# Ipsedo/MARLClassification

Hardware: NVIDIA B200
Metric: image_episodes_per_sec (higher is better)
Workload: dtype tf32x3

## Files before the change

include/marlc.h:

```cpp
#ifndef MARLC_H
#define MARLC_H
#include <stddef.h>
#include <stdint.h>
#ifdef __cplusplus
extern "C" {
#endif

#define MARLC_MAX_ACTIONS 16
#define MARLC_MAX_CNN_LAYERS 6

int marlc_version(void);
const char* marlc_last_error(void);
long marlc_selftest_fastdiv(int d_max, int stride);


int marlc_patch_gather(const float* img, const int64_t* pos, float* obs, int Na, int B, int C, int H, int W, int f,
                       void* stream);
int marlc_patch_gather_backward(const float* d_obs, const int64_t* pos, float* d_img, int Na, int B, int C, int H,
                                int W, int f, void* stream);

int marlc_transition(int64_t* pos, const int64_t* act, const int64_t* table, int nA, int M, int f, int H, int W,
                     float* norm_pos, int* err_flag, void* stream);

int marlc_normalized_positions(const int64_t* pos, float* out, int M, int H, int W, void* stream);
// ... 39 lines not shown
} marlc_config;

typedef struct marlc_engine marlc_engine;

int marlc_engine_create(const marlc_config* cfg, marlc_engine** out);
void marlc_engine_destroy(marlc_engine* e);

typedef struct marlc_plan {
    int cnn_wide;
    int cnn_nw;
    int cnn_batches;
    int cnn_ctas;
    int cnn_passes;
    int cnn_tail;
    int lstm_tc;
    int lstm_hu;
    int lstm_bn;
    int lstm_fat;
    int lstm_ks;
    int lstm_ksplit;
    int lstm_tail_rows;
    int sweep_chained;
    int staged_step_pre, staged_step_post, staged_bwd_pre, staged_bwd_post;
} marlc_plan;
int marlc_engine_plan(const marlc_engine* e, marlc_plan* out);

int marlc_engine_param_count(const marlc_engine* e);
int marlc_engine_param_info(const marlc_engine* e, int idx, char* name, int64_t* offset, int* ndim, int64_t* shape);
int64_t marlc_engine_param_floats(const marlc_engine* e);

size_t marlc_engine_workspace_bytes(const marlc_engine* e);
int marlc_engine_bind(marlc_engine* e, void* workspace, float* params, float* grads);
int marlc_engine_buffer(const marlc_engine* e, const char* name, size_t* offset, size_t* nbytes);

int marlc_episode_forward(marlc_engine* e, const float* img, const int64_t* pos0, const float* const* hidden0,
                          const int64_t* actions, void* stream);
int marlc_model_step(marlc_engine* e, const float* patch, const float* msg, const float* npos,
                     const float* const* hidden, void* stream);
int marlc_engine_seed(marlc_engine* e, uint64_t seed, void* stream);

int marlc_loss_phase_a(marlc_engine* e, const int64_t* targets, void* stream);
int marlc_loss_phase_b(marlc_engine* e, void* stream);

int marlc_episode_backward(marlc_engine* e, const float* img, int accumulate, void* stream);

int marlc_episode_image_grad(marlc_engine* e, float* d_img, void* stream);
// ... 20 lines not shown
```

marlclassification_b200/_lib.py:

```python
from __future__ import annotations

import ctypes as C
import os

import torch

from . import _build

MAX_ACTIONS = 16
MAX_CNN_LAYERS = 6


class MarlcConfig(C.Structure):

    _fields_ = [
        ("na", C.c_int), ("nb", C.c_int), ("T", C.c_int), ("C", C.c_int), ("H", C.c_int), ("W", C.c_int),
        ("f", C.c_int), ("n_actions", C.c_int), ("actions", (C.c_int * 2) * MAX_ACTIONS),
        ("cnn_layers", C.c_int), ("cnn_cin", C.c_int * MAX_CNN_LAYERS), ("cnn_cout", C.c_int * MAX_CNN_LAYERS),
        ("cnn_groups", C.c_int * MAX_CNN_LAYERS),
        ("n_b", C.c_int), ("n_a", C.c_int), ("n_m", C.c_int), ("n_m_o", C.c_int), ("n_d", C.c_int),
        ("nl_b", C.c_int), ("nl_a", C.c_int), ("nb_class", C.c_int),
        ("gamma", C.c_float), ("use_tc", C.c_int), ("use_chains", C.c_int),
    ]


class MarlcPlan(C.Structure):

    _fields_ = [(name, C.c_int) for name in (
        "cnn_wide", "cnn_nw", "cnn_batches", "cnn_ctas", "cnn_passes", "cnn_tail",
        "lstm_tc", "lstm_hu", "lstm_bn", "lstm_fat", "lstm_ks", "lstm_ksplit", "lstm_tail_rows",
        "sweep_chained", "staged_step_pre", "staged_step_post", "staged_bwd_pre", "staged_bwd_post")]

    def as_dict(self) -> dict:
        return {name: getattr(self, name) for name, _ in self._fields_}


_P = C.c_void_p
_SIGS = {
    "marlc_version": (C.c_int, []),
    "marlc_selftest_fastdiv": (C.c_long, [C.c_int, C.c_int]),
    "marlc_last_error": (C.c_char_p, []),
    "marlc_patch_gather": (C.c_int, [_P, _P, _P] + [C.c_int] * 6 + [_P]),
    "marlc_patch_gather_backward": (C.c_int, [_P, _P, _P] + [C.c_int] * 6 + [_P]),
    "marlc_transition": (C.c_int, [_P, _P, _P] + [C.c_int] * 5 + [_P, _P, _P]),
    "marlc_normalized_positions": (C.c_int, [_P, _P, C.c_int, C.c_int, C.c_int, _P]),
    "marlc_images_u8_to_f32": (C.c_int, [_P, _P] + [C.c_int] * 5 + [_P]),
    "marlc_linear": (C.c_int, [_P, _P, _P, _P, C.c_int, C.c_int, C.c_int, _P]),
    "marlc_ln_silu": (C.c_int, [_P, _P, _P, _P, C.c_int, C.c_int, _P]),
    "marlc_msg_mean": (C.c_int, [_P, _P, C.c_int, C.c_int, C.c_int, _P]),
    "marlc_tc_gemm": (C.c_int, [_P, C.c_int64, C.c_int, _P, C.c_int64, C.c_int, _P, C.c_int64, _P, C.c_int64, C.c_int, _P,
                                _P, C.c_int64, C.c_int, C.c_int, C.c_int, C.c_int, C.c_int, C.c_int, _P]),
    "marlc_tc_lstm_pair": (C.c_int, [_P, C.c_int, C.c_int, C.c_int] + [C.POINTER(_P)] * 9 + [C.c_int, _P]),
    "marlc_split_lo": (C.c_int, [_P, _P, C.c_int64, _P]),
    "marlc_tc_lstm_pair_presplit": (C.c_int, [_P, _P, C.c_int, C.c_int, C.c_int] + [C.POINTER(_P)] * 13 + [_P]),
# ... 81 lines not shown
```

marlclassification_b200/csrc/chain.cu:

```cuda
#include <initializer_list>

#include <stdlib.h>

#include "chain.cuh"
#include "cnn_wide.cuh"

namespace marlc {

constexpr int RB = 4;
constexpr int CT = 256;
constexpr int WT_K = 16;
constexpr int WT_P = WT_K + 1;
constexpr float LN_EPS_C = 1e-5f;


__device__ void rb_linear(const float* xT, const float* __restrict__ W, const float* __restrict__ bias, float* ys,
                          int ldy, int N, int K, float* wt) {
    const int tid = threadIdx.x;
    const bool vec = ((K & 3) == 0) && (((uintptr_t)W & 15) == 0);
    for (int n0 = 0; n0 < N; n0 += CT) {
        float acc[RB];
#pragma unroll
        for (int r = 0; r < RB; ++r) acc[r] = 0.f;
        const int n = n0 + tid;
// ... 49 lines not shown
#pragma unroll
        for (int r = 0; r < RB; ++r) out[r * ldo + k] = acc[r];
    }
    __syncthreads();
}


__device__ __forceinline__ void stage_w(float* dst, const float* __restrict__ W, int N, int K, int P) {
    stage_rows(dst, W, N, K, P);
}
__host__ __device__ inline int odd_pitch(int K) { return K | 1; }

__device__ __forceinline__ bool stage_w_async(float* dst, const float* __restrict__ W, int N, int K) {
    if (((K & 3) != 0) || ((reinterpret_cast<uintptr_t>(W) & 15) != 0)) { stage_rows(dst, W, N, K, K); return false; }
    const int tot4 = (N * K) >> 2;
    const uint32_t d0 = (uint32_t)__cvta_generic_to_shared(dst);
    for (int i = threadIdx.x; i < tot4; i += CT)
        asm volatile("cp.async.cg.shared.global [%0], [%1], 16;" ::"r"(d0 + 16u * i), "l"(W + 4 * (long)i) : "memory");
    asm volatile("cp.async.commit_group;" ::: "memory");
    return true;
}
__device__ __forceinline__ void stage_wait_all() { asm volatile("cp.async.wait_group 0;" ::: "memory"); }

__device__ void rb_linear_s(const float* xT, const float* Ws, int P, const float* __restrict__ bias, float* ys, int ldy,
                            int N, int K) {
    for (int n = threadIdx.x; n < N; n += CT) {
        const float* w = Ws + n * P;
        float a0 = 0.f, a1 = 0.f, a2 = 0.f, a3 = 0.f;
#pragma unroll 4
        for (int k = 0; k < K; ++k) {
            const float wv = w[k];
            const float4 x = *reinterpret_cast<const float4*>(xT + k * RB);
            a0 = fmaf(wv, x.x, a0); a1 = fmaf(wv, x.y, a1); a2 = fmaf(wv, x.z, a2); a3 = fmaf(wv, x.w, a3);
        }
        const float b = bias ? bias[n] : 0.f;
        ys[n] = a0 + b; ys[ldy + n] = a1 + b; ys[2 * ldy + n] = a2 + b; ys[3 * ldy + n] = a3 + b;
    }
    __syncthreads();
}

__device__ void rb_dx_s(const float* dyT, const float* Ws, int P, float* out, int ldo, int N, int K) {
    for (int k = threadIdx.x; k < K; k += CT) {
        float a0 = 0.f, a1 = 0.f, a2 = 0.f, a3 = 0.f;
#pragma unroll 4
        for (int n = 0; n < N; ++n) {
            const float wv = Ws[n * P + k];
            const float4 d = *reinterpret_cast<const float4*>(dyT + n * RB);
            a0 = fmaf(wv, d.x, a0); a1 = fmaf(wv, d.y, a1); a2 = fmaf(wv, d.z, a2); a3 = fmaf(wv, d.w, a3);
        }
        out[k] = a0; out[ldo + k] = a1; out[2 * ldo + k] = a2; out[3 * ldo + k] = a3;
    }
    __syncthreads();
}

__device__ void rb_ln_silu(const float* ys, int ldy, int N, const float* __restrict__ gamma,
                           const float* __restrict__ beta, int rows_valid, long row0, float* pre_g, long ld_pre,
                           float* s_g, long ld_s, float* sT, float* s_lo = nullptr) {
    const int warp = threadIdx.x >> 5, lane = threadIdx.x & 31;
    if (warp < RB) {
        const int r = warp;
        if (r < rows_valid) {
            const float* y = ys + r * ldy;
            const float inv = 1.0f / (float)N;
            float s = 0.f;
            for (int n = lane; n < N; n += 32) s += y[n];
            const float mean = warp_sum(s) * inv;
            float v = 0.f;
            for (int n = lane; n < N; n += 32) { const float d = y[n] - mean; v += d * d; }
            const float rstd = 1.0f / sqrtf(warp_sum(v) * inv + LN_EPS_C);
            for (int n = lane; n < N; n += 32) {
                const float yv = y[n];
                if (pre_g) pre_g[(row0 + r) * ld_pre + n] = yv;
                const float o = siluf_((yv - mean) * rstd * gamma[n] + beta[n]);
                if (s_g) s_g[(row0 + r) * ld_s + n] = o;
                if (s_lo) s_lo[(row0 + r) * ld_s + n] = tf32_lo(o);
                if (sT) sT[n * RB + r] = o;
            }
        } else if (sT) {
            for (int n = lane; n < N; n += 32) sT[n * RB + r] = 0.f;
        }
    }
    __syncthreads();
}

__device__ void rb_ln_silu_bwd(float* ds, float* ypre, int ld, int N, const float* __restrict__ gamma,
                               const float* __restrict__ beta, int rows_valid, long row0, float* dy, float* dyT,
                               float* dy_g, long ld_dyg, float* dgamma, float* dbeta, float* dbias) {
    const int warp = threadIdx.x >> 5, lane = threadIdx.x & 31;
    if (warp < RB) {
        const int r = warp;
        float* y = ypre + r * ld;
        float* g = ds + r * ld;
        if (r < rows_valid) {
            const float inv = 1.0f / (float)N;
            float s = 0.f;
            for (int n = lane; n < N; n += 32) s += y[n];
            const float mean = warp_sum(s) * inv;
            float v = 0.f;
            for (int n = lane; n < N; n += 32) { const float d = y[n] - mean; v += d * d; }
            const float rstd = 1.0f / sqrtf(warp_sum(v) * inv + LN_EPS_C);
            float c1 = 0.f, c2 = 0.f;
            for (int n = lane; n < N; n += 32) {
// ... 68 lines not shown
}
static int maxw_of(std::initializer_list<int> v) {
    int m = 4;
    for (int x : v) m = max(m, x);
    return (m + 3) & ~3;
}
ChainStage step_pre_stage(int n_m, int n1, int n2, int nd) {
    const int maxw = maxw_of({n_m, n1, n2, nd});
    return {maxw, staged_floats(maxw, n1, odd_pitch(n_m), n2, odd_pitch(n1))};
}
ChainStage step_post_stage(int n1, int n2) {
    const int maxw = maxw_of({n1, n2});
    return {maxw, staged_floats(maxw, n2, odd_pitch(n1), 0, 0)};
}
ChainStage bwd_pre_stage(int n_m, int n1, int nb) {
    const int maxw = maxw_of({n_m, n1, nb});
    return {maxw, staged_floats(maxw, n_m, n1, n1, nb)};
}
ChainStage bwd_post_stage(int n_m, int n1, int n2) {
    const int maxw = maxw_of({n_m, n1, n2});
    return {maxw, staged_floats(maxw, n2, n1, n1, n_m)};
}

struct StepPreWideArgs { StepPreArgs a; int maxw; int staged; int cnn_blocks; int dec_blocks; int trig; CnnWidePlan wide; };

__global__ void __launch_bounds__(CT, 1) step_pre_wide_kernel(const StepPreWideArgs ka) {
    extern __shared__ __align__(16) float sm[];
    const StepPreArgs& a = ka.a;
    if (ka.trig) pdl_trigger();
    if ((int)blockIdx.x < ka.cnn_blocks) {
        cnn_fwd_wide(a.cnn, ka.wide, blockIdx.x, ka.cnn_blocks, sm);
        return;
    }
    const int db = (int)blockIdx.x - ka.cnn_blocks;
    const int nrb = (a.M + RB - 1) / RB;
    const int n_m = a.d0.n_in, n1 = a.d0.n_out, n2 = a.d3.n_out;
    ChainSmem S(sm, ka.maxw);
    const int P0 = odd_pitch(n_m), P3 = odd_pitch(n1);
    float* W0s = S.wres;
    float* W3s = W0s + n1 * P0;
    const int tid = threadIdx.x;
    const bool fast = ka.staged && RB * n_m <= CT && n1 <= CT && n2 <= CT && 2 * (n1 + n2) <= CT * WT_P;
    float* sG0 = S.wt;
    float* sB0 = sG0 + n1;
    float* sG3 = sB0 + n1;
    float* sB3 = sG3 + n2;
    const int mr = tid / n_m, mj = tid - mr * n_m;
    auto load_mean = [&](int rb) -> float {
        const int row0 = rb * RB;
        return (tid < RB * n_m && rb < nrb && row0 + mr < a.M) ? other_agents_mean(a.msg_in, row0 + mr, mj, a.Na, a.Nb, n_m) : 0.f;
    };
    if (fast) {
        float g0 = 0.f, b0 = 0.f, g3 = 0.f, b3 = 0.f;
        if (tid < n1) { g0 = a.d0.g[tid]; b0 = a.d0.be[tid]; }
        if (tid < n2) { g3 = a.d3.g[tid]; b3 = a.d3.be[tid]; }
        stage_w(W0s, a.d0.W, n1, n_m, P0);
        stage_w(W3s, a.d3.W, n2, n1, P3);
        if (tid < n1) { sG0[tid] = g0; sB0[tid] = b0; }
        if (tid < n2) { sG3[tid] = g3; sB3[tid] = b3; }
    } else if (ka.staged) {
        stage_w(W0s, a.d0.W, n1, n_m, P0);
        stage_w(W3s, a.d3.W, n2, n1, P3);
    }
    pdl_wait();
    float mv = fast ? load_mean(db) : 0.f;
    for (int rb = db; rb < nrb; rb += ka.dec_blocks) {
        const int row0 = rb * RB;
        const int rows_valid = min(RB, a.M - row0);
        if (fast) {
            if (tid < RB * n_m) {
                if (mr < rows_valid) a.coll[(long)(row0 + mr) * n_m + mj] = mv;
                S.bufT[mj * RB + mr] = mv;
            }
            __syncthreads();
            mv = load_mean(rb + ka.dec_blocks);
            rb_linear_s(S.bufT, W0s, P0, a.d0.b, S.bufA, ka.maxw, n1, n_m);
            rb_ln_silu(S.bufA, ka.maxw, n1, sG0, sB0, rows_valid, row0, a.dec_y1, n1, a.dec_s1, n1, S.bufT);
            rb_linear_s(S.bufT, W3s, P3, a.d3.b, S.bufA, ka.maxw, n2, n1);
            rb_ln_silu(S.bufA, ka.maxw, n2, sG3, sB3, rows_valid, row0, a.dec_y2, n2, a.U + a.F, a.ldu, nullptr,
                       a.U_lo ? a.U_lo + a.F : nullptr);
        } else {
            for (int e = tid; e < RB * n_m; e += CT) {
                const int r = e / n_m, j = e % n_m;
                float v = 0.f;
                if (r < rows_valid) {
                    v = other_agents_mean(a.msg_in, row0 + r, j, a.Na, a.Nb, n_m);
                    a.coll[(long)(row0 + r) * n_m + j] = v;
                }
                S.bufT[j * RB + r] = v;
            }
            __syncthreads();
            if (ka.staged) rb_linear_s(S.bufT, W0s, P0, a.d0.b, S.bufA, ka.maxw, n1, n_m);
            else rb_linear(S.bufT, a.d0.W, a.d0.b, S.bufA, ka.maxw, n1, n_m, S.wt);
            rb_ln_silu(S.bufA, ka.maxw, n1, a.d0.g, a.d0.be, rows_valid, row0, a.dec_y1, n1, a.dec_s1, n1, S.bufT);
            if (ka.staged) rb_linear_s(S.bufT, W3s, P3, a.d3.b, S.bufA, ka.maxw, n2, n1);
            else rb_linear(S.bufT, a.d3.W, a.d3.b, S.bufA, ka.maxw, n2, n1, S.wt);
            rb_ln_silu(S.bufA, ka.maxw, n2, a.d3.g, a.d3.be, rows_valid, row0, a.dec_y2, n2, a.U + a.F, a.ldu, nullptr,
                       a.U_lo ? a.U_lo + a.F : nullptr);
        }
        {
            const int warp = tid >> 5, lane = tid & 31, nd = a.pos.n_out;
            if (warp < rows_valid) {
                const long m = row0 + warp;
                const float p0 = a.npos[2 * m], p1 = a.npos[2 * m + 1];
                const float inv = 1.0f / (float)nd;
                float sum = 0.f;
                for (int j = lane; j < nd; j += 32) {
                    const float y = fmaf(p1, a.pos.W[2 * j + 1], p0 * a.pos.W[2 * j]) + a.pos.b[j];
                    a.pos_y[m * nd + j] = y;
                    S.bufB[warp * ka.maxw + j] = y;
                    sum += y;
                }
                const float mean = warp_sum(sum) * inv;
                float v = 0.f;
                for (int j = lane; j < nd; j += 32) { const float d = S.bufB[warp * ka.maxw + j] - mean; v += d * d; }
                const float rstd = 1.0f / sqrtf(warp_sum(v) * inv + LN_EPS_C);
                float* o = a.U + m * a.ldu + a.F + n2;
                float* ol = a.U_lo ? a.U_lo + m * a.ldu + a.F + n2 : nullptr;
                for (int j = lane; j < nd; j += 32) {
                    const float v2 = siluf_((S.bufB[warp * ka.maxw + j] - mean) * rstd * a.pos.g[j] + a.pos.be[j]);
                    o[j] = v2;
                    if (ol) ol[j] = tf32_lo(v2);
                }
            }
        }
        __syncthreads();
    }
}

static int persistent_blocks(int nrb, size_t smem_bytes, int waves = 1) {
    const int per_sm = (int)max((size_t)1, min((size_t)8, (size_t)(220 * 1024) / max(smem_bytes, (size_t)1)));
    return max(1, min(nrb, MARLC_SMS * per_sm * waves));
}

static int step_pre_small(const StepPreArgs& a, cudaStream_t s);

constexpr int CNN_WIDE_MIN = 256;
StepPrePlan step_pre_plan(const CnnDesc& d, bool have_img, bool have_wT, int M, CnnWidePlan* wide) {
    CnnWidePlan w;
    memset(&w, 0, sizeof(w));
    if (M >= CNN_WIDE_MIN) w = cnn_wide_plan(d, have_img, have_wT);
    if (wide) *wide = w;
    StepPrePlan p;
    p.nw = w.ok ? CW_NW : 1;
    p.cnn_blocks = w.ok ? min((M + CW_NW - 1) / CW_NW, MARLC_SMS) : 0;
    return p;
}

int step_pre(const StepPreArgs& a, cudaStream_t s) {
    if (a.M <= 0) return 0;
    static_assert(CW_THREADS == CT, "the wide feature extractor runs inside the chain kernel's CTA shape");
    StepPreWideArgs ka;
    const StepPrePlan pl = step_pre_plan(a.cnn.d, a.cnn.img != nullptr && a.cnn.patch == nullptr, true, a.M, &ka.wide);
    if (!ka.wide.ok) return step_pre_small(a, s);
    ka.a = a;
    const ChainStage st = step_pre_stage(a.d0.n_in, a.d0.n_out, a.d3.n_out, a.pos.n_out);
    ka.maxw = st.maxw;
    const int wfl = st.wfl;
    ka.staged = wfl > 0;
    ka.cnn_blocks = pl.cnn_blocks;
    const size_t smem = max(chain_smem_bytes(ka.maxw) + sizeof(float) * (size_t)wfl, sizeof(float) * (size_t)ka.wide.smem_floats);
    MARLC_CHECK(smem <= 226 * 1024, "step_pre: shared memory %zu B too large", smem);
    static size_t attr = 0;
    if (smem > 48 * 1024 && smem > attr) {
        MARLC_CUDA(cudaFuncSetAttribute(step_pre_wide_kernel, cudaFuncAttributeMaxDynamicSharedMemorySize, (int)smem));
        attr = smem;
    }
    ka.dec_blocks = persistent_blocks((a.M + RB - 1) / RB, smem);
    const int grid = ka.cnn_blocks + ka.dec_blocks;
    ka.trig = pdl_trigger_early();
    MARLC_CUDA(launch_pdl(step_pre_wide_kernel, dim3(grid), dim3(CT), smem, s, ka));
    MARLC_LAUNCH_CHECK();
    return 0;
}

struct StepPreKernelArgs { StepPreArgs a; int maxw; int staged; int trig; };

__global__ void __launch_bounds__(CT) step_pre_kernel(const StepPreKernelArgs ka) {
    extern __shared__ __align__(16) float sm[];
    const StepPreArgs& a = ka.a;
    if (ka.trig) pdl_trigger();
    if ((int)blockIdx.x < a.M) {
        cnn_fwd_block(a.cnn, blockIdx.x, sm);
        return;
    }
    const int row0 = ((int)blockIdx.x - a.M) * RB;
    const int rows_valid = min(RB, a.M - row0);
    const int n_m = a.d0.n_in, n1 = a.d0.n_out, n2 = a.d3.n_out;
    ChainSmem S(sm, ka.maxw);
    const int P0 = odd_pitch(n_m), P3 = odd_pitch(n1);
    float* W0s = S.wres;
    float* W3s = W0s + n1 * P0;
    if (ka.staged && RB * n_m <= CT && n1 <= CT && n2 <= CT && 2 * (n1 + n2) <= CT * WT_P) {
        float* sG0 = S.wt;
// ... 197 lines not shown
    if (lane == 0) {
        float pa = 0.f;
        for (int j = 0; j < p.nA; ++j) {
            const float pr = logit[j] * invd;
            p.probs[(long)m * p.nA + j] = pr;
            if (j == act) pa = pr;
        }
        p.logp[m] = logf(pa);
        p.act_out[m] = act;
        int py = p.pos_in[2 * m], px = p.pos_in[2 * m + 1];
        if (act >= 0 && act < p.nA) {
            const int ny = py + p.moves[2 * act], nx = px + p.moves[2 * act + 1];
            if ((ny >= 0) & (ny + p.f < p.H) & (nx >= 0) & (nx + p.f < p.W)) { py = ny; px = nx; }
        }
        p.pos_out[2 * m] = py; p.pos_out[2 * m + 1] = px;
        p.step_pos[2 * (long)m] = py; p.step_pos[2 * (long)m + 1] = px;
        p.npos_out[2 * m] = (float)py / (float)p.H;
        p.npos_out[2 * m + 1] = (float)px / (float)p.W;
    }
}

struct StepPostKernelArgs { StepPostArgs a; int maxw; int pol_blocks; int staged; int trig; };

__global__ void __launch_bounds__(CT) step_post_kernel(const StepPostKernelArgs ka) {
    extern __shared__ __align__(16) float sm[];
    const StepPostArgs& a = ka.a;
    if (ka.trig) pdl_trigger();
    if ((int)blockIdx.x < ka.pol_blocks) {
        const int warp = threadIdx.x >> 5;
        const int m = blockIdx.x * (CT / 32) + warp;
        pdl_wait();
        if (m < a.M) policy_tail_row(a, m, sm + warp * a.act.nl);
        return;
    }
    const int row0 = ((int)blockIdx.x - ka.pol_blocks) * RB;
    const int rows_valid = min(RB, a.M - row0);
    const int n1 = a.e3.n_in, n2 = a.e3.n_out;
    ChainSmem S(sm, ka.maxw);
    const int P3 = odd_pitch(n1);
    if (ka.staged && RB * n1 <= 2 * CT && n1 <= CT && n2 <= CT && 2 * (n1 + n2) <= CT * WT_P) {
        float* sG1 = S.wt;
        float* sB1 = sG1 + n1;
        float* sG3 = sB1 + n1;
        float* sB3 = sG3 + n2;
        const int tid = threadIdx.x;
        float y1v[2] = {0.f, 0.f};
        int r1[2], k1[2];
#pragma unroll
        for (int i = 0; i < 2; ++i) { const int e = tid + i * CT; r1[i] = e / n1; k1[i] = e - r1[i] * n1; }
        pdl_wait();
#pragma unroll
        for (int i = 0; i < 2; ++i)
            if (r1[i] < rows_valid) y1v[i] = a.enc_y1[(long)(row0 + r1[i]) * n1 + k1[i]];
        float g1 = 0.f, b1 = 0.f, g3 = 0.f, b3 = 0.f;
        if (tid < n1) { g1 = a.enc_g[tid]; b1 = a.enc_be[tid]; }
// ... 3 lines not shown
        if (tid < n2) { sG3[tid] = g3; sB3[tid] = b3; }
#pragma unroll
        for (int i = 0; i < 2; ++i)
            if (r1[i] < RB) S.bufA[r1[i] * ka.maxw + k1[i]] = y1v[i];
        __syncthreads();
        rb_ln_silu(S.bufA, ka.maxw, n1, sG1, sB1, rows_valid, row0, nullptr, 0, a.enc_s1, n1, S.bufT);
        rb_linear_s(S.bufT, S.wres, P3, a.e3.b, S.bufA, ka.maxw, n2, n1);
        rb_ln_silu(S.bufA, ka.maxw, n2, sG3, sB3, rows_valid, row0, a.enc_y2, n2, a.msg_out, n2, nullptr);
        return;
    }
    if (ka.staged) stage_w(S.wres, a.e3.W, n2, n1, P3);
    pdl_wait();
    for (int e = threadIdx.x; e < RB * n1; e += CT) {
        const int r = e / n1, k = e % n1;
        S.bufA[r * ka.maxw + k] = r < rows_valid ? a.enc_y1[(long)(row0 + r) * n1 + k] : 0.f;
    }
    __syncthreads();
    rb_ln_silu(S.bufA, ka.maxw, n1, a.enc_g, a.enc_be, rows_valid, row0, nullptr, 0, a.enc_s1, n1, S.bufT);
    if (ka.staged) rb_linear_s(S.bufT, S.wres, P3, a.e3.b, S.bufA, ka.maxw, n2, n1);
    else rb_linear(S.bufT, a.e3.W, a.e3.b, S.bufA, ka.maxw, n2, n1, S.wt);
    rb_ln_silu(S.bufA, ka.maxw, n2, a.e3.g, a.e3.be, rows_valid, row0, a.enc_y2, n2, a.msg_out, n2, nullptr);
}

int step_post(const StepPostArgs& a, cudaStream_t s) {
    if (a.M <= 0) return 0;
    MARLC_CHECK(a.act.nA <= MAX_ACT, "step_post: nb_action=%d > %d", a.act.nA, MAX_ACT);
    StepPostKernelArgs ka;
    ka.a = a;
    const ChainStage st = step_post_stage(a.e3.n_in, a.e3.n_out);
    ka.maxw = st.maxw;
    ka.pol_blocks = (a.M + CT / 32 - 1) / (CT / 32);
    const int wfl = st.wfl;
    ka.staged = wfl > 0;
    const size_t smem = max(chain_smem_bytes(ka.maxw) + sizeof(float) * (size_t)wfl, sizeof(float) * (size_t)(CT / 32) * a.act.nl);
    MARLC_CHECK(smem <= 200 * 1024, "step_post: shared memory %zu B too large", smem);
    static size_t attr = 0;
    if (smem > 48 * 1024 && smem > attr) {
        MARLC_CUDA(cudaFuncSetAttribute(step_post_kernel, cudaFuncAttributeMaxDynamicSharedMemorySize, (int)smem));
        attr = smem;
    }
    const int grid = ka.pol_blocks + (a.M + RB - 1) / RB;
    ka.trig = pdl_trigger_early();
    MARLC_CUDA(launch_pdl(step_post_kernel, dim3(grid), dim3(CT), smem, s, ka));
    MARLC_LAUNCH_CHECK();
    return 0;
}


__device__ __forceinline__ void cell_bwd_rows(const int row0, const int rows_valid, const int n,
                                              const float* __restrict__ gates, const float* __restrict__ dh_heads,
                                              const float* __restrict__ dh_carry, const float* __restrict__ dc_next,
                                              const float* __restrict__ c_prev, const float* __restrict__ c_new,
                                              const float* dhx, const int ldx, float* __restrict__ dgates,
                                              float* __restrict__ dgates_lo, float* __restrict__ dc_prev) {
    for (int j = threadIdx.x; j < n; j += CT) {
        float gi[RB], gf[RB], gg[RB], go[RB], dh[RB], dcn[RB], cp[RB], cn[RB];
#pragma unroll
        for (int r = 0; r < RB; ++r) {
            if (r < rows_valid) {
                const long m = row0 + r, idx = m * n + j;
                const float* g = gates + m * 4 * n;
                gi[r] = g[j]; gf[r] = g[n + j]; gg[r] = g[2 * n + j]; go[r] = g[3 * n + j];
                dh[r] = dh_heads[idx] + (dh_carry ? dh_carry[idx] : 0.f);
                dcn[r] = dc_next ? dc_next[idx] : 0.f;
                cp[r] = c_prev[idx]; cn[r] = c_new[idx];
            }
        }
#pragma unroll
// ... 358 lines not shown
```

marlclassification_b200/csrc/chain.cuh:

```cuda
#pragma once
#include "cnn_device.cuh"
#include "kernels.cuh"

namespace marlc {

struct ChainLin {
    const float* W;
    const float* b;
    const float* g;
    const float* be;
    float* dW;
    float* db;
    float* dg;
    float* dbe;
    int n_in, n_out;
};

struct StepPreArgs {
    CnnFwdArgs cnn;
    const float* msg_in;
    float* coll;
    ChainLin d0, d3;
    float* dec_y1;
    float* dec_s1;
// ... 41 lines not shown
    float* dgates[2];
    float* dgates_lo[2] = {nullptr, nullptr};
    float* dc_prev[2];
    int n[2];
    int Na, Nb, M, n_m;
};
int bwd_pre(const BwdPreArgs& a, cudaStream_t s);

struct BwdPostArgs {
    const float* dU;
    long ldu;
    int F;
    ChainLin d0, d3;
    const float* dec_y1;
    const float* dec_y2;
    float* d_dec_y1;
    float* d_dec_y2;
    float* dcoll;
    int M, n_m, n_m_o;
};
int bwd_post(const BwdPostArgs& a, cudaStream_t s);

struct CnnWidePlan;
struct StepPrePlan { int nw, cnn_blocks; };
StepPrePlan step_pre_plan(const CnnDesc& d, bool have_img, bool have_wT, int M, CnnWidePlan* wide = nullptr);
struct ChainStage { int maxw, wfl; };
ChainStage step_pre_stage(int n_m, int n1, int n2, int nd);
ChainStage step_post_stage(int n1, int n2);
ChainStage bwd_pre_stage(int n_m, int n1, int nb);
ChainStage bwd_post_stage(int n_m, int n1, int n2);

}
```

marlclassification_b200/csrc/engine.cu:

```cuda
#include <stdarg.h>
#include <string.h>

#include <algorithm>

#include <string>
#include <vector>

#include <nvtx3/nvToolsExt.h>

#include "../../include/marlc.h"
#include "kernels.cuh"
#include "chain.cuh"
#include "tc.cuh"

namespace marlc {

int g_launch_count = 0;
long g_simt_gemm_launches = 0, g_tc_gemm_launches = 0;
static thread_local char g_err[512] = "";
void set_error(const char* fmt, ...) {
    va_list ap;
    va_start(ap, fmt);
    vsnprintf(g_err, sizeof(g_err), fmt, ap);
    va_end(ap);
// ... 394 lines not shown
    a.src[0] = e->P; a.dst[0] = e->buf("params_lo"); a.n[0] = e->param_floats;
    a.src[1] = h0; a.dst[1] = h0 ? e->buf("H_lo") + (h0 - e->buf("H")) : nullptr; a.n[1] = h0 ? (long)e->M * e->cfg.n_b : 0;
    a.src[2] = hc0; a.dst[2] = hc0 ? e->buf("Hc_lo") + (hc0 - e->buf("Hc")) : nullptr; a.n[2] = hc0 ? (long)e->M * e->cfg.n_a : 0;
    split_lo_kernel<<<dim3(296, 3), 256, 0, s>>>(a);
    MARLC_LAUNCH_CHECK();
    return 0;
}

static inline int x3_of(const marlc_engine* e) { return e->cfg.use_tc == 2 ? 1 : 0; }

static bool lstm_on_tc(const marlc_engine* e) {
    const marlc_config& c = e->cfg;
    return c.use_tc && c.n_a == c.n_b && tc_lstm_shapes_ok(e->Kin, c.n_b);
}
constexpr int SWEEP_UNFUSED_MIN_M = 4096;
static bool sweep_chained(const marlc_engine* e) { return e->cfg.use_chains && e->M < SWEEP_UNFUSED_MIN_M; }

extern "C" int marlc_engine_plan(const marlc_engine* e, marlc_plan* out) {
    MARLC_CHECK(e && out, "plan: null argument");
    const marlc_config& c = e->cfg;
    const int M = e->M;
    marlc_plan p;
    memset(&p, 0, sizeof(p));
    const StepPrePlan sp = c.use_chains ? step_pre_plan(e->cnn, true, true, M) : StepPrePlan{1, 0};
    p.cnn_wide = sp.cnn_blocks > 0;
    p.cnn_nw = sp.nw;
    p.cnn_batches = (M + sp.nw - 1) / sp.nw;
    p.cnn_ctas = p.cnn_wide ? sp.cnn_blocks : M;
    p.cnn_passes = (p.cnn_batches + p.cnn_ctas - 1) / p.cnn_ctas;
    p.cnn_tail = M - (p.cnn_batches - 1) * sp.nw;
    if (lstm_on_tc(e)) {
        const TcLstmPlan lp = tc_lstm_plan(M, c.n_b, c.n_a, x3_of(e) != 0);
        p.lstm_tc = 1;
        p.lstm_hu = lp.hu; p.lstm_bn = lp.bn; p.lstm_fat = lp.fat; p.lstm_ks = lp.ks; p.lstm_ksplit = lp.ksplit;
        p.lstm_tail_rows = lp.tail_rows;
    }
    p.sweep_chained = sweep_chained(e);
    if (c.use_chains) {
        p.staged_step_pre = step_pre_stage(c.n_m, 2 * c.n_m, c.n_m_o, c.n_d).wfl > 0;
        p.staged_step_post = step_post_stage(2 * c.n_m, c.n_m).wfl > 0;
    }
    if (p.sweep_chained) {
        p.staged_bwd_pre = bwd_pre_stage(c.n_m, 2 * c.n_m, c.n_b).wfl > 0;
        p.staged_bwd_post = bwd_post_stage(c.n_m, 2 * c.n_m, c.n_m_o).wfl > 0;
    }
    *out = p;
    return 0;
}
static bool tc_worth(int m_out, int n_out, int k_red) { return n_out >= 16 && k_red >= 32 && m_out >= 1; }

static int G_nt(const marlc_engine* e, const float* X, long ldx, const float* W, long ldw, const float* bias, float* Y,
                long ldy, int M, int N, int K, int accumulate, cudaStream_t s) {
    if (e->cfg.use_tc && tc_worth(M, N, K)) {
        TcGemmArgs a;
        a.A = tc_op(X, ldx); a.B = tc_op(W, ldw); a.K = K;
        a.C = Y; a.ldc = ldy; a.M = M; a.N = N; a.bias = bias; a.accumulate = accumulate;
        a.x3 = x3_of(e);
        if (tc_operand_ok(a.A) && tc_operand_ok(a.B)) return tc_gemm(a, s);
    }
    return gemm_nt(X, ldx, W, ldw, bias, Y, ldy, M, N, K, accumulate, s);
}
static int G_nn(const marlc_engine* e, const float* dY, long lddy, const float* W, long ldw, float* dX, long lddx, int M,
                int N, int K, int accumulate, cudaStream_t s) {
// ... 1065 lines not shown
```

Measured before the change: 20000.

## Process 32-row blocks in decoder/encoder chains and schedule decoder work onto CNN CTAs

Row-block linear and LN/SiLU helpers are templated on the row count so the step_pre decoder and the step_post encoder can process 32 rows per CTA with a padded transposed tile and multiple output columns per thread. This raises weight reuse per shared-memory load. A new decoder schedule places row blocks on spare CTAs and on CNN CTAs after their CNN work finishes, replacing the separate persistent decoder grid. The trade-off is more shared memory per CTA and a more complex schedule that could load-imbalance or reduce occupancy.

```diff
diff --git a/include/marlc.h b/include/marlc.h
--- a/include/marlc.h
+++ b/include/marlc.h
@@ -85,6 +85,9 @@
     int lstm_tail_rows;
     int sweep_chained;
     int staged_step_pre, staged_step_post, staged_bwd_pre, staged_bwd_post;
+    int dec_rows;
+    int dec_in_cnn;
+    int post_rows;
 } marlc_plan;
 int marlc_engine_plan(const marlc_engine* e, marlc_plan* out);
 
diff --git a/marlclassification_b200/_lib.py b/marlclassification_b200/_lib.py
--- a/marlclassification_b200/_lib.py
+++ b/marlclassification_b200/_lib.py
@@ -29,7 +29,8 @@
     _fields_ = [(name, C.c_int) for name in (
         "cnn_wide", "cnn_nw", "cnn_batches", "cnn_ctas", "cnn_passes", "cnn_tail",
         "lstm_tc", "lstm_hu", "lstm_bn", "lstm_fat", "lstm_ks", "lstm_ksplit", "lstm_tail_rows",
-        "sweep_chained", "staged_step_pre", "staged_step_post", "staged_bwd_pre", "staged_bwd_post")]
+        "sweep_chained", "staged_step_pre", "staged_step_post", "staged_bwd_pre", "staged_bwd_post",
+        "dec_rows", "dec_in_cnn", "post_rows")]
 
     def as_dict(self) -> dict:
         return {name: getattr(self, name) for name, _ in self._fields_}
diff --git a/marlclassification_b200/csrc/chain.cu b/marlclassification_b200/csrc/chain.cu
--- a/marlclassification_b200/csrc/chain.cu
+++ b/marlclassification_b200/csrc/chain.cu
@@ -95,21 +95,55 @@
 }
 __device__ __forceinline__ void stage_wait_all() { asm volatile("cp.async.wait_group 0;" ::: "memory"); }
 
+template <int R>
+__host__ __device__ constexpr int xt_pitch() { return R == RB ? RB : R + 4; }
+
+template <int R, int NT>
+__device__ __forceinline__ void rb_linear_tile(const float* xT, const float* Ws, int P, const float* __restrict__ bias,
+                                               float* ys, int ldy, int N, int K) {
+    constexpr int TPG = CT / (R / 4), XP = xt_pitch<R>();
+    const int g = R == RB ? 0 : (int)threadIdx.x / TPG, c = R == RB ? (int)threadIdx.x : (int)threadIdx.x % TPG;
+    const float* x = xT + 4 * g;
+    for (int n0 = c; n0 < N; n0 += NT * TPG) {
+        const float* w[NT];
+        float acc[NT][4];
+#pragma unroll
+        for (int j = 0; j < NT; ++j) {
+            const int n = n0 + j * TPG;
+            w[j] = Ws + (NT == 1 || n < N ? n : n0) * P;
+            acc[j][0] = 0.f; acc[j][1] = 0.f; acc[j][2] = 0.f; acc[j][3] = 0.f;
+        }
+#pragma unroll 4
+        for (int k = 0; k < K; ++k) {
+            const float4 xv = *reinterpret_cast<const float4*>(x + k * XP);
+#pragma unroll
+            for (int j = 0; j < NT; ++j) {
+                const float wv = w[j][k];
+                acc[j][0] = fmaf(wv, xv.x, acc[j][0]); acc[j][1] = fmaf(wv, xv.y, acc[j][1]);
+                acc[j][2] = fmaf(wv, xv.z, acc[j][2]); acc[j][3] = fmaf(wv, xv.w, acc[j][3]);
+            }
+        }
+#pragma unroll
+        for (int j = 0; j < NT; ++j) {
+            const int n = n0 + j * TPG;
+            if (NT == 1 || n < N) {
+                const float b = bias ? bias[n] : 0.f;
+                float* y = ys + 4 * g * ldy + n;
+                y[0] = acc[j][0] + b; y[ldy] = acc[j][1] + b; y[2 * ldy] = acc[j][2] + b; y[3 * ldy] = acc[j][3] + b;
+            }
+        }
+    }
+    __syncthreads();
+}
+
+template <int R = RB>
 __device__ void rb_linear_s(const float* xT, const float* Ws, int P, const float* __restrict__ bias, float* ys, int ldy,
                             int N, int K) {
-    for (int n = threadIdx.x; n < N; n += CT) {
-        const float* w = Ws + n * P;
-        float a0 = 0.f, a1 = 0.f, a2 = 0.f, a3 = 0.f;
-#pragma unroll 4
-        for (int k = 0; k < K; ++k) {
-            const float wv = w[k];
-            const float4 x = *reinterpret_cast<const float4*>(xT + k * RB);
-            a0 = fmaf(wv, x.x, a0); a1 = fmaf(wv, x.y, a1); a2 = fmaf(wv, x.z, a2); a3 = fmaf(wv, x.w, a3);
-        }
-        const float b = bias ? bias[n] : 0.f;
-        ys[n] = a0 + b; ys[ldy + n] = a1 + b; ys[2 * ldy + n] = a2 + b; ys[3 * ldy + n] = a3 + b;
-    }
-    __syncthreads();
+    constexpr int TPG = CT / (R / 4);
+    if constexpr (R == RB) rb_linear_tile<R, 1>(xT, Ws, P, bias, ys, ldy, N, K);
+    else if (N <= 2 * TPG) rb_linear_tile<R, 2>(xT, Ws, P, bias, ys, ldy, N, K);
+    else if (N <= 3 * TPG) rb_linear_tile<R, 3>(xT, Ws, P, bias, ys, ldy, N, K);
+    else rb_linear_tile<R, 4>(xT, Ws, P, bias, ys, ldy, N, K);
 }
 
 __device__ void rb_dx_s(const float* dyT, const float* Ws, int P, float* out, int ldo, int N, int K) {
@@ -126,10 +160,12 @@
     __syncthreads();
 }
 
+template <int R = RB>
 __device__ void rb_ln_silu(const float* ys, int ldy, int N, const float* __restrict__ gamma,
                            const float* __restrict__ beta, int rows_valid, long row0, float* pre_g, long ld_pre,
                            float* s_g, long ld_s, float* sT, float* s_lo = nullptr) {
     const int warp = threadIdx.x >> 5, lane = threadIdx.x & 31;
+    if constexpr (R == RB) {
     if (warp < RB) {
         const int r = warp;
         if (r < rows_valid) {
@@ -151,6 +187,40 @@
             }
         } else if (sT) {
             for (int n = lane; n < N; n += 32) sT[n * RB + r] = 0.f;
+        }
+    }
+    } else {
+        constexpr int RPW = R / (CT / 32), XP = xt_pitch<R>();
+        const float inv = 1.0f / (float)N;
+        float s[RPW], mean[RPW], v[RPW], rstd[RPW];
+#pragma unroll
+        for (int i = 0; i < RPW; ++i) { s[i] = 0.f; v[i] = 0.f; }
+        for (int n = lane; n < N; n += 32)
+#pragma unroll
+            for (int i = 0; i < RPW; ++i) s[i] += ys[(warp + 8 * i) * ldy + n];
+#pragma unroll
+        for (int i = 0; i < RPW; ++i) mean[i] = warp_sum(s[i]) * inv;
+        for (int n = lane; n < N; n += 32)
+#pragma unroll
+            for (int i = 0; i < RPW; ++i) { const float d = ys[(warp + 8 * i) * ldy + n] - mean[i]; v[i] += d * d; }
+#pragma unroll
+        for (int i = 0; i < RPW; ++i) rstd[i] = 1.0f / sqrtf(warp_sum(v[i]) * inv + LN_EPS_C);
+        for (int n = lane; n < N; n += 32) {
+            const float ga = gamma[n], be = beta[n];
+#pragma unroll
+            for (int i = 0; i < RPW; ++i) {
+                const int r = warp + 8 * i;
+                if (r < rows_valid) {
+                    const float yv = ys[r * ldy + n];
+                    if (pre_g) pre_g[(row0 + r) * ld_pre + n] = yv;
+                    const float o = siluf_((yv - mean[i]) * rstd[i] * ga + be);
+                    if (s_g) s_g[(row0 + r) * ld_s + n] = o;
+                    if (s_lo) s_lo[(row0 + r) * ld_s + n] = tf32_lo(o);
+                    if (sT) sT[n * XP + r] = o;
+                } else if (sT) {
+                    sT[n * XP + r] = 0.f;
+                }
+            }
         }
     }
     __syncthreads();
@@ -265,115 +335,163 @@
     return {maxw, staged_floats(maxw, n2, n1, n1, n_m)};
 }
 
-struct StepPreWideArgs { StepPreArgs a; int maxw; int staged; int cnn_blocks; int dec_blocks; int trig; CnnWidePlan wide; };
+constexpr int ROWS_R = 32;
+
+__host__ __device__ inline int round4(int n) { return (n + 3) & ~3; }
+static int rows_smem_floats(int maxw, int wfl, int naff) {
+    return round4(wfl) + round4(naff) + ROWS_R * maxw + maxw * xt_pitch<ROWS_R>();
+}
+static int rows_staged_floats(int maxw, int naff, int n1, int p1, int n2, int p2) {
+    const int w = n1 * p1 + n2 * p2;
+    return sizeof(float) * (size_t)rows_smem_floats(maxw, w, naff) <= CHAIN_SMEM_LIMIT ? w : 0;
+}
+struct RowsSmem {
+    float *w, *aff, *ys, *xT;
+    __device__ RowsSmem(float* sm, int maxw, int wfl, int naff) {
+        w = sm; aff = w + round4(wfl); ys = aff + round4(naff); xT = ys + ROWS_R * maxw;
+    }
+};
+
+template <int R>
+__device__ void rb_stage_mean(const StepPreArgs& a, const int row0, const int rows_valid, float* xT) {
+    constexpr int U = 8, XP = xt_pitch<R>();
+    const int n = a.d0.n_in, Na = a.Na;
+    const long stride = (long)a.Nb * n;
+    for (int e0 = threadIdx.x; e0 < R * n; e0 += U * CT) {
+        int r[U], j[U];
+        bool ok[U];
+        const float* base[U];
+        float s[U];
+#pragma unroll
+        for (int u = 0; u < U; ++u) {
+            const int e = e0 + u * CT;
+            r[u] = e / n; j[u] = e - r[u] * n;
+            ok[u] = e < R * n && r[u] < rows_valid && Na > 1;
+            base[u] = a.msg_in + (long)((row0 + r[u]) % a.Nb) * n + j[u];
+            s[u] = 0.f;
+        }
+        int ag = 0;
+        for (; ag + 8 <= Na; ag += 8) {
+            float v[U][8];
+#pragma unroll
+            for (int u = 0; u < U; ++u)
+#pragma unroll
+                for (int i = 0; i < 8; ++i) v[u][i] = ok[u] ? base[u][(ag + i) * stride] : 0.f;
+#pragma unroll
+            for (int u = 0; u < U; ++u)
+                s[u] += ((v[u][0] + v[u][1]) + (v[u][2] + v[u][3])) + ((v[u][4] + v[u][5]) + (v[u][6] + v[u][7]));
+        }
+        for (; ag < Na; ++ag)
+#pragma unroll
+            for (int u = 0; u < U; ++u) s[u] += ok[u] ? base[u][ag * stride] : 0.f;
+#pragma unroll
+        for (int u = 0; u < U; ++u) {
+            const float v = ok[u] ? (s[u] - a.msg_in[(long)(row0 + r[u]) * n + j[u]]) / (float)(Na - 1) : 0.f;
+            if (e0 + u * CT < R * n) {
+                if (r[u] < rows_valid) a.coll[(long)(row0 + r[u]) * n + j[u]] = v;
+                xT[j[u] * XP + r[u]] = v;
+            }
+        }
+    }
+    __syncthreads();
+}
+
+__device__ void rb_pos_features(const StepPreArgs& a, const int row0, const int rows_valid, float* ybuf, int ldy) {
+    const int warp = threadIdx.x >> 5, lane = threadIdx.x & 31, nd = a.pos.n_out, n2 = a.d3.n_out;
+    for (int r = warp; r < rows_valid; r += CT / 32) {
+        const long m = row0 + r;
+        float* yb = ybuf + r * ldy;
+        const float p0 = a.npos[2 * m], p1 = a.npos[2 * m + 1];
+        const float inv = 1.0f / (float)nd;
+        float sum = 0.f;
+        for (int j = lane; j < nd; j += 32) {
+            const float y = fmaf(p1, a.pos.W[2 * j + 1], p0 * a.pos.W[2 * j]) + a.pos.b[j];
+            a.pos_y[m * nd + j] = y;
+            yb[j] = y;
+            sum += y;
+        }
+        const float mean = warp_sum(sum) * inv;
+        float v = 0.f;
+        for (int j = lane; j < nd; j += 32) { const float d = yb[j] - mean; v += d * d; }
+        const float rstd = 1.0f / sqrtf(warp_sum(v) * inv + LN_EPS_C);
+        float* o = a.U + m * a.ldu + a.F + n2;
+        float* ol = a.U_lo ? a.U_lo + m * a.ldu + a.F + n2 : nullptr;
+        for (int j = lane; j < nd; j += 32) {
+            const float v2 = siluf_((yb[j] - mean) * rstd * a.pos.g[j] + a.pos.be[j]);
+            o[j] = v2;
+            if (ol) ol[j] = tf32_lo(v2);
+        }
+    }
+    __syncthreads();
+}
+
+constexpr int DEC_BLOCKS_PER_BATCH = 3;
+
+static DecSched dec_sched(int M, int nbatch, int cnn_blocks) {
+    DecSched d;
+    d.rows = ROWS_R;
+    d.nrb = (M + ROWS_R - 1) / ROWS_R;
+    if (cnn_blocks == MARLC_SMS) {
+        const int rem = nbatch % cnn_blocks;
+        d.grid = cnn_blocks;
+        d.spare0 = rem ? rem : cnn_blocks;
+    } else {
+        d.grid = cnn_blocks + max(1, min(MARLC_SMS - cnn_blocks, d.nrb));
+        d.spare0 = cnn_blocks;
+    }
+    d.slots = (d.grid - d.spare0) * DEC_BLOCKS_PER_BATCH;
+    d.in_cnn = d.spare0 < cnn_blocks || d.nrb > d.slots;
+    return d;
+}
+
+struct StepPreWideArgs { StepPreArgs a; int maxw; int wfl; int cnn_blocks; DecSched ds; int trig; CnnWidePlan wide; };
 
 __global__ void __launch_bounds__(CT, 1) step_pre_wide_kernel(const StepPreWideArgs ka) {
     extern __shared__ __align__(16) float sm[];
     const StepPreArgs& a = ka.a;
+    const DecSched& ds = ka.ds;
     if (ka.trig) pdl_trigger();
-    if ((int)blockIdx.x < ka.cnn_blocks) {
-        cnn_fwd_wide(a.cnn, ka.wide, blockIdx.x, ka.cnn_blocks, sm);
+    const int cta = blockIdx.x;
+    const int spare_end = min(ds.slots, ds.nrb), nspare = ds.grid - ds.spare0;
+    const int first_spare = cta >= ds.spare0 && cta - ds.spare0 < spare_end ? cta - ds.spare0 : -1;
+    const bool any = first_spare >= 0 || ds.slots + cta < ds.nrb;
+    if (cta < ka.cnn_blocks) {
+        cnn_fwd_wide(a.cnn, ka.wide, cta, ka.cnn_blocks, sm);
+        if (!any) return;
+        __syncthreads();
+    } else if (!any) {
         return;
     }
-    const int db = (int)blockIdx.x - ka.cnn_blocks;
-    const int nrb = (a.M + RB - 1) / RB;
-    const int n_m = a.d0.n_in, n1 = a.d0.n_out, n2 = a.d3.n_out;
-    ChainSmem S(sm, ka.maxw);
-    const int P0 = odd_pitch(n_m), P3 = odd_pitch(n1);
-    float* W0s = S.wres;
-    float* W3s = W0s + n1 * P0;
-    const int tid = threadIdx.x;
-    const bool fast = ka.staged && RB * n_m <= CT && n1 <= CT && n2 <= CT && 2 * (n1 + n2) <= CT * WT_P;
-    float* sG0 = S.wt;
+    const int n_m = a.d0.n_in, n1 = a.d0.n_out, n2 = a.d3.n_out, mw = ka.maxw;
+    RowsSmem S(sm, mw, ka.wfl, 2 * (n1 + n2));
+    const bool staged = ka.wfl > 0;
+    const int P0 = staged ? odd_pitch(n_m) : n_m, P3 = staged ? odd_pitch(n1) : n1;
+    const float* W0 = staged ? S.w : a.d0.W;
+    const float* W3 = staged ? S.w + n1 * P0 : a.d3.W;
+    float* sG0 = S.aff;
     float* sB0 = sG0 + n1;
     float* sG3 = sB0 + n1;
     float* sB3 = sG3 + n2;
-    const int mr = tid / n_m, mj = tid - mr * n_m;
-    auto load_mean = [&](int rb) -> float {
-        const int row0 = rb * RB;
-        return (tid < RB * n_m && rb < nrb && row0 + mr < a.M) ? other_agents_mean(a.msg_in, row0 + mr, mj, a.Na, a.Nb, n_m) : 0.f;
+    if (staged) {
+        stage_w(S.w, a.d0.W, n1, n_m, P0);
+        stage_w(S.w + n1 * P0, a.d3.W, n2, n1, P3);
+    }
+    for (int i = threadIdx.x; i < n1; i += CT) { sG0[i] = a.d0.g[i]; sB0[i] = a.d0.be[i]; }
+    for (int i = threadIdx.x; i < n2; i += CT) { sG3[i] = a.d3.g[i]; sB3[i] = a.d3.be[i]; }
+    pdl_wait();
+    auto block = [&](int rb) {
+        const int row0 = rb * ROWS_R, rows_valid = min(ROWS_R, a.M - row0);
+        rb_stage_mean<ROWS_R>(a, row0, rows_valid, S.xT);
+        rb_linear_s<ROWS_R>(S.xT, W0, P0, a.d0.b, S.ys, mw, n1, n_m);
+        rb_ln_silu<ROWS_R>(S.ys, mw, n1, sG0, sB0, rows_valid, row0, a.dec_y1, n1, a.dec_s1, n1, S.xT);
+        rb_linear_s<ROWS_R>(S.xT, W3, P3, a.d3.b, S.ys, mw, n2, n1);
+        rb_ln_silu<ROWS_R>(S.ys, mw, n2, sG3, sB3, rows_valid, row0, a.dec_y2, n2, a.U + a.F, a.ldu, nullptr,
+                           a.U_lo ? a.U_lo + a.F : nullptr);
+        rb_pos_features(a, row0, rows_valid, S.ys, mw);
     };
-    if (fast) {
-        float g0 = 0.f, b0 = 0.f, g3 = 0.f, b3 = 0.f;
-        if (tid < n1) { g0 = a.d0.g[tid]; b0 = a.d0.be[tid]; }
-        if (tid < n2) { g3 = a.d3.g[tid]; b3 = a.d3.be[tid]; }
-        stage_w(W0s, a.d0.W, n1, n_m, P0);
-        stage_w(W3s, a.d3.W, n2, n1, P3);
-        if (tid < n1) { sG0[tid] = g0; sB0[tid] = b0; }
-        if (tid < n2) { sG3[tid] = g3; sB3[tid] = b3; }
-    } else if (ka.staged) {
-        stage_w(W0s, a.d0.W, n1, n_m, P0);
-        stage_w(W3s, a.d3.W, n2, n1, P3);
-    }
-    pdl_wait();
-    float mv = fast ? load_mean(db) : 0.f;
-    for (int rb = db; rb < nrb; rb += ka.dec_blocks) {
-        const int row0 = rb * RB;
-        const int rows_valid = min(RB, a.M - row0);
-        if (fast) {
-            if (tid < RB * n_m) {
-                if (mr < rows_valid) a.coll[(long)(row0 + mr) * n_m + mj] = mv;
-                S.bufT[mj * RB + mr] = mv;
-            }
-            __syncthreads();
-            mv = load_mean(rb + ka.dec_blocks);
-            rb_linear_s(S.bufT, W0s, P0, a.d0.b, S.bufA, ka.maxw, n1, n_m);
-            rb_ln_silu(S.bufA, ka.maxw, n1, sG0, sB0, rows_valid, row0, a.dec_y1, n1, a.dec_s1, n1, S.bufT);
-            rb_linear_s(S.bufT, W3s, P3, a.d3.b, S.bufA, ka.maxw, n2, n1);
-            rb_ln_silu(S.bufA, ka.maxw, n2, sG3, sB3, rows_valid, row0, a.dec_y2, n2, a.U + a.F, a.ldu, nullptr,
-                       a.U_lo ? a.U_lo + a.F : nullptr);
-        } else {
-            for (int e = tid; e < RB * n_m; e += CT) {
-                const int r = e / n_m, j = e % n_m;
-                float v = 0.f;
-                if (r < rows_valid) {
-                    v = other_agents_mean(a.msg_in, row0 + r, j, a.Na, a.Nb, n_m);
-                    a.coll[(long)(row0 + r) * n_m + j] = v;
-                }
-                S.bufT[j * RB + r] = v;
-            }
-            __syncthreads();
-            if (ka.staged) rb_linear_s(S.bufT, W0s, P0, a.d0.b, S.bufA, ka.maxw, n1, n_m);
-            else rb_linear(S.bufT, a.d0.W, a.d0.b, S.bufA, ka.maxw, n1, n_m, S.wt);
-            rb_ln_silu(S.bufA, ka.maxw, n1, a.d0.g, a.d0.be, rows_valid, row0, a.dec_y1, n1, a.dec_s1, n1, S.bufT);
-            if (ka.staged) rb_linear_s(S.bufT, W3s, P3, a.d3.b, S.bufA, ka.maxw, n2, n1);
-            else rb_linear(S.bufT, a.d3.W, a.d3.b, S.bufA, ka.maxw, n2, n1, S.wt);
-            rb_ln_silu(S.bufA, ka.maxw, n2, a.d3.g, a.d3.be, rows_valid, row0, a.dec_y2, n2, a.U + a.F, a.ldu, nullptr,
-                       a.U_lo ? a.U_lo + a.F : nullptr);
-        }
-        {
-            const int warp = tid >> 5, lane = tid & 31, nd = a.pos.n_out;
-            if (warp < rows_valid) {
-                const long m = row0 + warp;
-                const float p0 = a.npos[2 * m], p1 = a.npos[2 * m + 1];
-                const float inv = 1.0f / (float)nd;
-                float sum = 0.f;
-                for (int j = lane; j < nd; j += 32) {
-                    const float y = fmaf(p1, a.pos.W[2 * j + 1], p0 * a.pos.W[2 * j]) + a.pos.b[j];
-                    a.pos_y[m * nd + j] = y;
-                    S.bufB[warp * ka.maxw + j] = y;
-                    sum += y;
-                }
-                const float mean = warp_sum(sum) * inv;
-                float v = 0.f;
-                for (int j = lane; j < nd; j += 32) { const float d = S.bufB[warp * ka.maxw + j] - mean; v += d * d; }
-                const float rstd = 1.0f / sqrtf(warp_sum(v) * inv + LN_EPS_C);
-                float* o = a.U + m * a.ldu + a.F + n2;
-                float* ol = a.U_lo ? a.U_lo + m * a.ldu + a.F + n2 : nullptr;
-                for (int j = lane; j < nd; j += 32) {
-                    const float v2 = siluf_((S.bufB[warp * ka.maxw + j] - mean) * rstd * a.pos.g[j] + a.pos.be[j]);
-                    o[j] = v2;
-                    if (ol) ol[j] = tf32_lo(v2);
-                }
-            }
-        }
-        __syncthreads();
-    }
-}
-
-static int persistent_blocks(int nrb, size_t smem_bytes, int waves = 1) {
-    const int per_sm = (int)max((size_t)1, min((size_t)8, (size_t)(220 * 1024) / max(smem_bytes, (size_t)1)));
-    return max(1, min(nrb, MARLC_SMS * per_sm * waves));
+    if (first_spare >= 0)
+        for (int rb = first_spare; rb < spare_end; rb += nspare) block(rb);
+    for (int rb = ds.slots + cta; rb < ds.nrb; rb += ds.grid) block(rb);
 }
 
 static int step_pre_small(const StepPreArgs& a, cudaStream_t s);
@@ -385,8 +503,11 @@
     if (M >= CNN_WIDE_MIN) w = cnn_wide_plan(d, have_img, have_wT);
     if (wide) *wide = w;
     StepPrePlan p;
+    memset(&p, 0, sizeof(p));
     p.nw = w.ok ? CW_NW : 1;
     p.cnn_blocks = w.ok ? min((M + CW_NW - 1) / CW_NW, MARLC_SMS) : 0;
+    if (w.ok) p.dec = dec_sched(M, (M + CW_NW - 1) / CW_NW, p.cnn_blocks);
+    else p.dec.rows = RB;
     return p;
 }
 
@@ -397,22 +518,21 @@
     const StepPrePlan pl = step_pre_plan(a.cnn.d, a.cnn.img != nullptr && a.cnn.patch == nullptr, true, a.M, &ka.wide);
     if (!ka.wide.ok) return step_pre_small(a, s);
     ka.a = a;
-    const ChainStage st = step_pre_stage(a.d0.n_in, a.d0.n_out, a.d3.n_out, a.pos.n_out);
-    ka.maxw = st.maxw;
-    const int wfl = st.wfl;
-    ka.staged = wfl > 0;
+    const int n_m = a.d0.n_in, n1 = a.d0.n_out, n2 = a.d3.n_out;
+    ka.maxw = maxw_of({n_m, n1, n2, a.pos.n_out});
+    const int naff = 2 * (n1 + n2);
+    ka.wfl = rows_staged_floats(ka.maxw, naff, n1, odd_pitch(n_m), n2, odd_pitch(n1));
     ka.cnn_blocks = pl.cnn_blocks;
-    const size_t smem = max(chain_smem_bytes(ka.maxw) + sizeof(float) * (size_t)wfl, sizeof(float) * (size_t)ka.wide.smem_floats);
+    ka.ds = pl.dec;
+    const size_t smem = sizeof(float) * (size_t)max(rows_smem_floats(ka.maxw, ka.wfl, naff), ka.wide.smem_floats);
     MARLC_CHECK(smem <= 226 * 1024, "step_pre: shared memory %zu B too large", smem);
     static size_t attr = 0;
     if (smem > 48 * 1024 && smem > attr) {
         MARLC_CUDA(cudaFuncSetAttribute(step_pre_wide_kernel, cudaFuncAttributeMaxDynamicSharedMemorySize, (int)smem));
         attr = smem;
     }
-    ka.dec_blocks = persistent_blocks((a.M + RB - 1) / RB, smem);
-    const int grid = ka.cnn_blocks + ka.dec_blocks;
     ka.trig = pdl_trigger_early();
-    MARLC_CUDA(launch_pdl(step_pre_wide_kernel, dim3(grid), dim3(CT), smem, s, ka));
+    MARLC_CUDA(launch_pdl(step_pre_wide_kernel, dim3(ka.ds.grid), dim3(CT), smem, s, ka));
     MARLC_LAUNCH_CHECK();
     return 0;
 }
@@ -656,6 +776,33 @@
 
 struct StepPostKernelArgs { StepPostArgs a; int maxw; int pol_blocks; int staged; int trig; };
 
+__device__ void enc_rows_block(const StepPostKernelArgs& ka, const int rb, float* sm) {
+    const StepPostArgs& a = ka.a;
+    const int n1 = a.e3.n_in, n2 = a.e3.n_out, mw = ka.maxw;
+    const int row0 = rb * ROWS_R, rows_valid = min(ROWS_R, a.M - row0);
+    RowsSmem S(sm, mw, ka.staged, 2 * (n1 + n2));
+    const int P3 = ka.staged ? odd_pitch(n1) : n1;
+    float* sG1 = S.aff;
+    float* sB1 = sG1 + n1;
+    float* sG3 = sB1 + n1;
+    float* sB3 = sG3 + n2;
+    if (ka.staged) stage_w(S.w, a.e3.W, n2, n1, P3);
+    for (int i = threadIdx.x; i < n1; i += CT) { sG1[i] = a.enc_g[i]; sB1[i] = a.enc_be[i]; }
+    for (int i = threadIdx.x; i < n2; i += CT) { sG3[i] = a.e3.g[i]; sB3[i] = a.e3.be[i]; }
+    pdl_wait();
+#pragma unroll 4
+    for (int e = threadIdx.x; e < rows_valid * n1; e += CT) {
+        const int r = e / n1, k = e - r * n1;
+        S.ys[r * mw + k] = a.enc_y1[(long)row0 * n1 + e];
+    }
+    __syncthreads();
+    rb_ln_silu<ROWS_R>(S.ys, mw, n1, sG1, sB1, rows_valid, row0, nullptr, 0, a.enc_s1, n1, S.xT);
+    rb_linear_s<ROWS_R>(S.xT, ka.staged ? S.w : a.e3.W, P3, a.e3.b, S.ys, mw, n2, n1);
+    rb_ln_silu<ROWS_R>(S.ys, mw, n2, sG3, sB3, rows_valid, row0, a.enc_y2, n2, a.msg_out, n2, nullptr);
+}
+
+
+template <int R>
 __global__ void __launch_bounds__(CT) step_post_kernel(const StepPostKernelArgs ka) {
     extern __shared__ __align__(16) float sm[];
     const StepPostArgs& a = ka.a;
@@ -665,6 +812,10 @@
         const int m = blockIdx.x * (CT / 32) + warp;
         pdl_wait();
         if (m < a.M) policy_tail_row(a, m, sm + warp * a.act.nl);
+        return;
+    }
+    if constexpr (R != RB) {
+        enc_rows_block(ka, (int)blockIdx.x - ka.pol_blocks, sm);
         return;
     }
     const int row0 = ((int)blockIdx.x - ka.pol_blocks) * RB;
@@ -714,6 +865,24 @@
     rb_ln_silu(S.bufA, ka.maxw, n2, a.e3.g, a.e3.be, rows_valid, row0, a.enc_y2, n2, a.msg_out, n2, nullptr);
 }
 
+constexpr int POST_ROWS_MIN_M = 1024;
+int step_post_rows(int M) { return M >= POST_ROWS_MIN_M ? ROWS_R : RB; }
+
+template <int R>
+static int step_post_launch(StepPostKernelArgs& ka, size_t smem, cudaStream_t s) {
+    MARLC_CHECK(smem <= 200 * 1024, "step_post: shared memory %zu B too large", smem);
+    static size_t attr = 0;
+    if (smem > 48 * 1024 && smem > attr) {
+        MARLC_CUDA(cudaFuncSetAttribute(step_post_kernel<R>, cudaFuncAttributeMaxDynamicSharedMemorySize, (int)smem));
+        attr = smem;
+    }
+    const int grid = ka.pol_blocks + (ka.a.M + R - 1) / R;
+    ka.trig = pdl_trigger_early();
+    MARLC_CUDA(launch_pdl(step_post_kernel<R>, dim3(grid), dim3(CT), smem, s, ka));
+    MARLC_LAUNCH_CHECK();
+    return 0;
+}
+
 int step_post(const StepPostArgs& a, cudaStream_t s) {
     if (a.M <= 0) return 0;
     MARLC_CHECK(a.act.nA <= MAX_ACT, "step_post: nb_action=%d > %d", a.act.nA, MAX_ACT);
@@ -722,20 +891,15 @@
     const ChainStage st = step_post_stage(a.e3.n_in, a.e3.n_out);
     ka.maxw = st.maxw;
     ka.pol_blocks = (a.M + CT / 32 - 1) / (CT / 32);
+    const size_t pol_smem = sizeof(float) * (size_t)(CT / 32) * a.act.nl;
+    if (step_post_rows(a.M) == ROWS_R) {
+        const int n1 = a.e3.n_in, n2 = a.e3.n_out, naff = 2 * (n1 + n2);
+        ka.staged = rows_staged_floats(ka.maxw, naff, n2, odd_pitch(n1), 0, 0);
+        return step_post_launch<ROWS_R>(ka, max(sizeof(float) * (size_t)rows_smem_floats(ka.maxw, ka.staged, naff), pol_smem), s);
+    }
     const int wfl = st.wfl;
     ka.staged = wfl > 0;
-    const size_t smem = max(chain_smem_bytes(ka.maxw) + sizeof(float) * (size_t)wfl, sizeof(float) * (size_t)(CT / 32) * a.act.nl);
-    MARLC_CHECK(smem <= 200 * 1024, "step_post: shared memory %zu B too large", smem);
-    static size_t attr = 0;
-    if (smem > 48 * 1024 && smem > attr) {
-        MARLC_CUDA(cudaFuncSetAttribute(step_post_kernel, cudaFuncAttributeMaxDynamicSharedMemorySize, (int)smem));
-        attr = smem;
-    }
-    const int grid = ka.pol_blocks + (a.M + RB - 1) / RB;
-    ka.trig = pdl_trigger_early();
-    MARLC_CUDA(launch_pdl(step_post_kernel, dim3(grid), dim3(CT), smem, s, ka));
-    MARLC_LAUNCH_CHECK();
-    return 0;
+    return step_post_launch<RB>(ka, max(chain_smem_bytes(ka.maxw) + sizeof(float) * (size_t)wfl, pol_smem), s);
 }
 
 
diff --git a/marlclassification_b200/csrc/chain.cuh b/marlclassification_b200/csrc/chain.cuh
--- a/marlclassification_b200/csrc/chain.cuh
+++ b/marlclassification_b200/csrc/chain.cuh
@@ -87,10 +87,12 @@
 int bwd_post(const BwdPostArgs& a, cudaStream_t s);
 
 struct CnnWidePlan;
-struct StepPrePlan { int nw, cnn_blocks; };
+struct DecSched { int rows, nrb, grid, spare0, slots, in_cnn; };
+struct StepPrePlan { int nw, cnn_blocks; DecSched dec; };
 StepPrePlan step_pre_plan(const CnnDesc& d, bool have_img, bool have_wT, int M, CnnWidePlan* wide = nullptr);
 struct ChainStage { int maxw, wfl; };
 ChainStage step_pre_stage(int n_m, int n1, int n2, int nd);
+int step_post_rows(int M);
 ChainStage step_post_stage(int n1, int n2);
 ChainStage bwd_pre_stage(int n_m, int n1, int nb);
 ChainStage bwd_post_stage(int n_m, int n1, int n2);
diff --git a/marlclassification_b200/csrc/engine.cu b/marlclassification_b200/csrc/engine.cu
--- a/marlclassification_b200/csrc/engine.cu
+++ b/marlclassification_b200/csrc/engine.cu
@@ -440,7 +440,7 @@
     const int M = e->M;
     marlc_plan p;
     memset(&p, 0, sizeof(p));
-    const StepPrePlan sp = c.use_chains ? step_pre_plan(e->cnn, true, true, M) : StepPrePlan{1, 0};
+    const StepPrePlan sp = c.use_chains ? step_pre_plan(e->cnn, true, true, M) : StepPrePlan{1, 0, {}};
     p.cnn_wide = sp.cnn_blocks > 0;
     p.cnn_nw = sp.nw;
     p.cnn_batches = (M + sp.nw - 1) / sp.nw;
@@ -457,6 +457,9 @@
     if (c.use_chains) {
         p.staged_step_pre = step_pre_stage(c.n_m, 2 * c.n_m, c.n_m_o, c.n_d).wfl > 0;
         p.staged_step_post = step_post_stage(2 * c.n_m, c.n_m).wfl > 0;
+        p.dec_rows = sp.dec.rows;
+        p.dec_in_cnn = sp.dec.in_cnn;
+        p.post_rows = step_post_rows(M);
     }
     if (p.sweep_chained) {
         p.staged_bwd_pre = bwd_pre_stage(c.n_m, 2 * c.n_m, c.n_b).wfl > 0;
```

New measurement: 19530 (median of 6 runs). 0.977x the previous value.
